# NekoImageLand/retto

Measured on AMD Instinct MI355X. Metric: images/sec end-to-end PP-OCRv4 det+rec @960x960, higher is better.
Workload: dtype f32; 1 GPU; C3: PP-OCRv4 mobile det+cls+rec full pipeline, batch=32 pages of 960x960 per GPU, 32 planted lines/page (planted DB map drives box extraction; det net fully executed, checksum 1.46374e+07); pages resident in HBM when the timed region starts; weights=seeded synthetic, PP-OCRv4 mobile shapes, networks=mobile/f32 f32 mobile/f32, parallelism=dp1 (pages sharded, no per-step collective), batches_in_flight=2

## Files before the change

include/retto_hip.h:

```cpp
#ifndef RETTO_HIP_H
#define RETTO_HIP_H

#include <stddef.h>
#include <stdint.h>

#ifdef __cplusplus
extern "C" {
#endif

#define RT_API __attribute__((visibility("default")))

typedef enum rt_status {
  RT_OK = 0,
  RT_ERR_IO = 1,
  RT_ERR_IMAGE = 2,
  RT_ERR_SHAPE = 3,
  RT_ERR_BACKEND = 4,
  RT_ERR_UTF8 = 5,
  RT_ERR_MODEL_NOT_FOUND = 7,
  RT_ERR_INVALID = 8,
  RT_ERR_CAPACITY = 9
} rt_status;

typedef struct rt_model_source {
// ... 294 lines not shown
                           int sh, int sw, const float* w, const float* bias, int act, int has_lab, float lab_a, float lab_c,
                           int pooled, int form, float* out, float* partial_out, long long partial_cap, float* mean_out,
                           int* info_out);
RT_API int rt_debug_attention(rt_session* s, const float* qkv, long long rows, const int* tokens, int n_lines, int heads,
                              float* out);
RT_API int rt_debug_lc_block(rt_session* s, const float* x, const int* heights, const int* widths, int n_img, int cin, int cout,
                             int sh, int sw, const float* dw_w, const float* dw_bias, const float* pw_w, const float* pw_bias,
                             int dw_act, int dw_has_lab, float dw_a, float dw_c, int pw_has_lab, float pw_a, float pw_c, int form,
                             float* out, int* info_out);
RT_API int rt_debug_dw_plan(int K, int sh, int sw, int Cp, int maxHo, int maxWo, int pooled, int form, int* plan_out);
RT_API int rt_debug_lc_wide(rt_session* s, const float* x, const int* heights, const int* widths, int n_img, int K, int cin, int cout,
                            int sh, int sw, const float* dw_w, const float* dw_bias, const float* pw_w, const float* pw_bias, int dw_act,
                            int dw_has_lab, float dw_a, float dw_c, int pw_has_lab, float pw_a, float pw_c, const float* fc1_w,
                            const float* fc1_b, const float* fc2_w, const float* fc2_b, int dw_form, float* out, long long out_len,
                            float* y1_out, long long y1_len, float* scale_out, long long scale_len, int* info_out);
RT_API int rt_debug_conv13(rt_session* s, const float* x, long long rows, int ldx, const int* tokens_per_line, int n_lines, int cin,
                           const float* w, int cout, const float* bias, int act, int form, float* out, int* info_out);
RT_API int rt_debug_layernorm(rt_session* s, const float* x, const float* r, long long rows, int C, const float* g,
                              const float* beta, float eps, float* out);
RT_API int rt_debug_glue16(rt_session* s, int op, const int* ip, const float* fp, const int* src_h, const int* src_w,
                           const int* dst_h, const int* dst_w, int n_img, const float* x, long long x_len, const float* x2,
                           long long x2_len, const float* tab, long long tab_len, float* out, long long out_len);
RT_API int rt_debug_fpn(rt_session* s, int op, const int* ip, const float* fp, const int* fine_h, const int* fine_w,
                        const int* coarse_h, const int* coarse_w, int n_img, const float* const* in, const long long* in_len,
                        float* const* out, const long long* out_len, int* info_out);
RT_API int rt_debug_conv16x(rt_session* s, const int* ip, const float* fp, const int* heights, const int* widths, int n_img,
                            const float* x, long long x_len, const float* wt, long long wt_len, const float* bias, const float* res,
                            long long res_len, const float* dot_w, float* out, long long out_len, int* route_out);
RT_API int rt_debug_cls_block(rt_session* s, const float* x, int n, int H, int W, int cin, int mid, int cout, int k, int sh, int act,
                              int se, const float* exp_w, const float* exp_b, const float* dw_w, const float* dw_b, const float* fc1_w,
// ... 17 lines not shown
```

retto_amd/_lib.py:

```python
from __future__ import annotations

import ctypes as C
import os

_HERE = os.path.dirname(os.path.abspath(__file__))
LIB_PATH = os.path.join(_HERE, "libretto_hip.so")

RT_OK = 0
RT_MEM_HOST, RT_MEM_DEVICE, RT_MEM_HOST_MAPS_DEVICE = 0, 1, 2
RT_MAX_INFLIGHT = 8
RT_DTYPE_F32, RT_DTYPE_F16 = 0, 1
STATUS_NAMES = {0: "OK", 1: "IOError", 2: "ImageError", 3: "ShapeError", 4: "BackendError", 5: "Utf8Error",
                7: "ModelNotFoundError", 8: "InvalidArgument", 9: "CapacityError"}


class ModelSource(C.Structure):
    _fields_ = [("path", C.c_char_p), ("data", C.c_void_p), ("len", C.c_size_t)]


class Config(C.Structure):
    _fields_ = [
        ("struct_size", C.c_uint32), ("device_id", C.c_int32),
        ("det", ModelSource), ("cls", ModelSource), ("rec", ModelSource), ("dict", ModelSource),
        ("max_side_len", C.c_int32), ("min_side_len", C.c_int32),
# ... 53 lines not shown

EXPORTS = [
    "rt_config_default", "rt_create", "rt_destroy", "rt_last_error", "rt_version",
    "rt_det", "rt_cls", "rt_rec", "rt_rec_ragged", "rt_rec_classes", "rt_model_info",
    "rt_resize_both_dims", "rt_resize_both", "rt_det_input_dims", "rt_det_preprocess", "rt_det_postprocess",
    "rt_crop_dims", "rt_crop_images", "rt_scale_and_clip", "rt_resize_norm_width", "rt_resize_norm_image",
    "rt_ctc_decode",
    "rt_run_batch", "rt_run_batch_stream", "rt_submit_batch", "rt_wait_batch", "rt_host_cpu_budget", "rt_results_free", "rt_results_pages", "rt_results_count", "rt_results_boxes",
    "rt_results_det_scores", "rt_results_cls_labels", "rt_results_cls_scores", "rt_results_rec_scores",
    "rt_results_rec_tokens", "rt_results_rec_text", "rt_results_rec_words", "rt_results_rec_word_text", "rt_debug_word_boxes", "rt_results_rec_candidates",
    "rt_debug_ctc_candidates", "rt_debug_ctc_candidates_host", "rt_results_det_checksum", "rt_results_json",
    "rt_device_malloc", "rt_device_free", "rt_memcpy_h2d", "rt_memcpy_d2h", "rt_synchronize",
    "rt_set_lanes", "rt_profile_enable", "rt_profile_get",
    "rt_onnx_to_rtwb", "rt_buffer_free", "rt_model_manifest", "rt_decode_image", "rt_run_encoded_batch",
    "rt_submit_encoded_batch", "rt_decode_batch", "rt_debug_jpeg_reconstruct",
    "rt_debug_set_variants", "rt_bench_gemm", "rt_bench_gemm_err", "rt_bench_lc", "rt_debug_conv16", "rt_debug_gemm", "rt_debug_dwconv", "rt_debug_dw_plan", "rt_debug_attention", "rt_debug_lc_block", "rt_debug_lc_wide", "rt_debug_conv13", "rt_debug_layernorm", "rt_debug_glue16", "rt_debug_conv16x", "rt_debug_fpn", "rt_debug_cls_block", "rt_debug_stem", "rt_debug_glue32", "rt_parse_dictionary", "rt_format_f32", "rt_rccl_unique_id", "rt_broadcast_blobs",
    "rt_run_regions", "rt_debug_warp_crops",
    "rt_charset_create", "rt_charset_classes", "rt_set_rec_charset", "rt_run_regions_charsets", "rt_debug_charset_compile",
    "rt_debug_ctc_charset", "rt_debug_ctc_charset_host",
    "rt_lexicon_create", "rt_lexicon_entries", "rt_lexicon_entry", "rt_lexicon_entry_text", "rt_set_rec_lexicon",
    "rt_run_regions_lexicons", "rt_results_rec_lexicon", "rt_results_rec_lexicon_id", "rt_debug_lexicon_compile",
    "rt_debug_ctc_lexicon", "rt_debug_ctc_lexicon_host",
    "rt_lexicon_set_snap", "rt_lexicon_snap", "rt_results_rec_lexicon_snapped", "rt_debug_ctc_lexicon_align",
    "rt_debug_ctc_lexicon_align_host",
    "rt_pattern_create", "rt_pattern_info", "rt_pattern_text", "rt_set_rec_pattern", "rt_run_regions_patterns", "rt_results_rec_pattern",
    "rt_debug_pattern_compile", "rt_debug_ctc_pattern", "rt_debug_ctc_pattern_host",
    "rt_keywords_create", "rt_keywords_entries", "rt_keywords_entry", "rt_keywords_entry_text", "rt_keywords_min_score",
    "rt_set_rec_keywords", "rt_run_regions_keywords", "rt_results_rec_keywords", "rt_results_rec_keywords_id", "rt_debug_ctc_keywords",
    "rt_debug_ctc_keywords_host", "rt_debug_span_quad",
    "rt_set_rec_beam", "rt_rec_beam", "rt_results_rec_beams", "rt_results_rec_beam_tokens", "rt_results_rec_beam_text",
    "rt_debug_ctc_beam", "rt_debug_ctc_beam_host",
# ... 109 lines not shown
                                        P(C.c_float), C.c_int, C.c_int, C.c_int, C.c_int, C.c_int, P(Word), P(C.c_int)]
    lib.rt_debug_gemm.argtypes = [C.c_void_p, C.c_void_p, C.c_longlong, C.c_int, C.c_int, C.c_void_p, C.c_int, C.c_void_p,
                                  C.c_int, C.c_int, C.c_float, C.c_float, C.c_void_p, C.c_int, C.c_void_p,
                                  C.c_int, C.c_void_p, C.c_int, C.c_int, C.c_int, C.c_int, C.c_int, C.c_int,
                                  C.c_void_p, C.c_void_p, C.c_void_p, C.c_void_p]
    lib.rt_debug_dwconv.argtypes = [C.c_void_p, C.c_void_p, C.c_void_p, C.c_void_p, C.c_int, C.c_int, C.c_int, C.c_int, C.c_int, C.c_int,
                                    C.c_void_p, C.c_void_p, C.c_int, C.c_int, C.c_float, C.c_float, C.c_int, C.c_int,
                                    C.c_void_p, C.c_void_p, C.c_longlong, C.c_void_p, C.c_void_p]
    lib.rt_debug_attention.argtypes = [C.c_void_p, C.c_void_p, C.c_longlong, C.c_void_p, C.c_int, C.c_int, C.c_void_p]
    lib.rt_debug_lc_block.argtypes = [C.c_void_p, C.c_void_p, C.c_void_p, C.c_void_p, C.c_int, C.c_int, C.c_int, C.c_int, C.c_int,
                                      C.c_void_p, C.c_void_p, C.c_void_p, C.c_void_p, C.c_int, C.c_int, C.c_float, C.c_float,
                                      C.c_int, C.c_float, C.c_float, C.c_int, C.c_void_p, C.c_void_p]
    lib.rt_debug_dw_plan.argtypes = [C.c_int] * 8 + [C.c_void_p]
    lib.rt_debug_lc_wide.argtypes = ([C.c_void_p] * 4 + [C.c_int] * 6 + [C.c_void_p] * 4 + [C.c_int, C.c_int, C.c_float, C.c_float, C.c_int,
                                     C.c_float, C.c_float] + [C.c_void_p] * 4 + [C.c_int] + [C.c_void_p, C.c_longlong] * 3 + [C.c_void_p])
    lib.rt_debug_conv13.argtypes = [C.c_void_p, C.c_void_p, C.c_longlong, C.c_int, C.c_void_p, C.c_int, C.c_int, C.c_void_p, C.c_int,
                                    C.c_void_p, C.c_int, C.c_int, C.c_void_p, C.c_void_p]
    lib.rt_debug_layernorm.argtypes = [C.c_void_p, C.c_void_p, C.c_void_p, C.c_longlong, C.c_int, C.c_void_p, C.c_void_p, C.c_float,
                                       C.c_void_p]
    lib.rt_debug_glue16.argtypes = [C.c_void_p, C.c_int, C.c_void_p, C.c_void_p, C.c_void_p, C.c_void_p, C.c_void_p, C.c_void_p, C.c_int,
                                    C.c_void_p, C.c_longlong, C.c_void_p, C.c_longlong, C.c_void_p, C.c_longlong, C.c_void_p,
                                    C.c_longlong]
    lib.rt_debug_fpn.argtypes = [C.c_void_p, C.c_int, C.c_void_p, C.c_void_p, C.c_void_p, C.c_void_p, C.c_void_p, C.c_void_p, C.c_int,
                                 C.c_void_p, C.c_void_p, C.c_void_p, C.c_void_p, C.c_void_p]
    lib.rt_debug_conv16x.argtypes = [C.c_void_p, C.c_void_p, C.c_void_p, C.c_void_p, C.c_void_p, C.c_int, C.c_void_p, C.c_longlong,
                                     C.c_void_p, C.c_longlong, C.c_void_p, C.c_void_p, C.c_longlong, C.c_void_p, C.c_void_p,
                                     C.c_longlong, C.c_void_p]
    lib.rt_debug_cls_block.argtypes = [C.c_void_p, C.c_void_p] + [C.c_int] * 10 + [C.c_void_p] * 10 + [C.c_int, C.c_void_p, C.c_void_p]
    lib.rt_debug_stem.argtypes = [C.c_void_p, C.c_void_p, C.c_void_p, C.c_void_p, C.c_void_p, C.c_int, C.c_int, C.c_void_p, C.c_void_p,
                                  C.c_int, C.c_float, C.c_void_p, C.c_void_p, C.c_void_p, C.c_longlong]
# ... 110 lines not shown
```

retto_amd/csrc/api_debug.cpp:

```cpp
#include <cmath>
#include <cstdio>
#include <cstdlib>
#include <cstring>

#include "api_internal.h"

using namespace rt;

namespace {
using nh::half_t;

std::vector<half_t> pack_conv16_weights(const float* wt, int cout, int cin, int kh, int kw, int cin_pad) {
  const int npad = round_up(cout, 32), nslab = (cin_pad + nh::KS - 1) / nh::KS;
  std::vector<half_t> hw((size_t)nslab * kh * kw * npad * nh::KS, (half_t)0.f);
  for (int n = 0; n < cout; n++)
    for (int k = 0; k < cin; k++)
      for (int t = 0; t < kh * kw; t++)
        hw[(((size_t)(k / nh::KS) * kh * kw + t) * npad + n) * nh::KS + k % nh::KS] = (half_t)wt[((size_t)n * cin + k) * kh * kw + t];
  return hw;
}

inline uint64_t xorshift64(uint64_t& s) { s ^= s << 13; s ^= s >> 7; s ^= s << 17; return s; }

template <typename F>
// ... 404 lines not shown
    DevBufs::download(out, dy, (size_t)out_n);
    DevBufs::download(y1_out, dy1, (size_t)y1_n);
    if (se) {
      const uint32_t cw = RT_DEBUG_CANARY;
      for (long long i = 0; i < scale_n; i++) memcpy(scale_out + i, &cw, 4);
      if (tr.scale) DevBufs::download(scale_out, tr.scale, (size_t)n_img * Cp);
    }
    const bool unfused = plan.route == nn::LC_UNFUSED;
    const int f[16] = {(int)plan.route, unfused ? (int)plan.dw.kernel : 0, unfused ? plan.dw.inst : plan.inst, plan.dw.R, plan.dw.lanes,
                       plan.dw.spb, plan.dw.chunks, (int)plan.dw.grid_x, (int)plan.dw.grid_z, plan.se_rows,
                       unfused ? (int)tr.gemm.kernel : 0, unfused && tr.gemm.se ? 1 : 0, tr.scale ? (tr.scaled_in_place ? 2 : 1) : 0, 0, 0, 0};
    memcpy(info_out, f, sizeof f);
  });
}

RT_API int rt_debug_conv13(rt_session* s, const float* x, long long rows, int ldx, const int* tokens_per_line, int n_lines, int cin,
                           const float* w, int cout, const float* bias, int act, int form, float* out, int* info_out) {
  RT_REQUIRE(s && x && tokens_per_line && w && out && info_out, s, "rt_debug_conv13: null argument");
  RT_REQUIRE(rows > 0 && rows < (1ll << 24) && n_lines > 0 && n_lines <= RT_MAX_GRID_Y && cin > 0 && cin % 4 == 0 && ldx >= cin &&
                 ldx % 4 == 0 && cout > 0 && cout <= 64 && act >= ACT_NONE && act <= ACT_SIGMOID && (form == 0 || form == 1),
             s, "rt_debug_conv13: bad shape");
  RT_REQUIRE(rows * ldx < (1ll << 30), s, "rt_debug_conv13: too large");
  for (int i = 0; i < n_lines; i++) RT_REQUIRE(tokens_per_line[i] > 0, s, "rt_debug_conv13: a line without tokens");
  const Ragged lines(tokens_per_line, n_lines);
  RT_REQUIRE(lines.total == rows, s, "rt_debug_conv13: the lines' tokens do not add up to rows");
  return guarded(s, [&] {
    RT_HIP_CHECK(hipSetDevice(s->device));
    WeightStore ws;
    const PackedDense pw = pack_conv(ws, w, bias, cout, cin, 1, 3);
    if (form == 1 && !nn::conv13_flat_supported(cout, pw.Npad)) throw RtError(RT_ERR_INVALID, "rt_debug_conv13: conv13_flat has no instance for the layer");
// ... 684 lines not shown
```

retto_amd/csrc/lc_plan.cpp:

```cpp
#include "lc_plan.h"

#include "gemm_plan.h"

namespace rt {
namespace nn {

int g_lc_wave = env_int("RT_LC_WAVE", 3);
int g_dw_sweep = env_int("RT_DW_SWEEP", 4);

namespace {

struct SweepInst { int K, sh, sw, min_ho, inst, inst_pooled; };
constexpr SweepInst SWEEPS[] = {{5, 1, 1, 5, 1, 3}, {3, 1, 1, 3, 2, 0}, {5, 2, 1, 3, 4, 5}, {3, 1, 2, 3, 6, 0}};

struct ThinInst { int sh, sw, c4, nt32, inst, th; };
constexpr ThinInst THINS[] = {{1, 1, 4, 1, 1, 8},  {1, 1, 8, 2, 2, 8},
                              {1, 1, 12, 2, 3, 4}, {1, 1, 16, 2, 4, 4},
                              {2, 2, 8, 2, 6, 4},  {2, 2, 12, 3, 7, 4}};
struct WaveInst { int sh, sw, Cp, Npad16, inst; };
constexpr WaveInst WAVES[] = {{1, 1, 16, 32, 1}, {1, 1, 32, 64, 2}, {1, 1, 48, 48, 3}, {1, 1, 64, 64, 4},
                              {2, 2, 32, 48, 6}, {2, 2, 48, 96, 7}, {2, 1, 64, 128, 8}};

int thin_inst(const LcShape& s, int* th) {
  if (s.K != 3 || s.Cp != round_up(s.C, 4)) return 0;
// ... 55 lines not shown
  };
  if (!s.se) {
    int th = 0;
    if (const int inst = g_lc_wave ? wave_inst(s, epi) : 0) {
      if (g_lc_wave >= 3 || inst >= 6) return fused(LC_LDS, inst, s.sh == 1 ? 4 : 2, 4 * LC_WAVE_TPW);
      return fused(LC_WAVE, inst, 2, 4 * LC_WAVE_TPW);
    }
    if (const int inst = thin_inst(s, &th)) return fused(LC_THIN, inst, th, LC_THIN_TPB);
  }
  if (s.se && (s.K == 3 || s.K == 5))
    p.se_rows = gemm_se_rows(s.Cp, s.rows, round_up(s.C, 4), s.N, s.Npad16, epi.act, s.min_pix);
  p.dw = dw_plan(s.K, s.sh, s.sw, s.Cp, s.maxHo, s.maxWo, p.se_rows > 0);
  return p;
}

}
}
```

retto_amd/csrc/lc_plan.h:

```cpp
#pragma once
#include "common.h"

namespace rt {
namespace nn {

extern int g_lc_wave;
extern int g_dw_sweep;

constexpr int DW_SWEEP_POOL_STRIPS = 4;
constexpr int LC_THIN_TPB = 8;
constexpr int LC_WAVE_TPW = 4;

constexpr int dw_rows_inst(int lanes, int K, int R, int sh, int sw) { return (((lanes * 8 + K) * 8 + R) * 4 + sh) * 4 + sw; }
enum class DwKernel {
  invalid,
  rows32,
  rows64,
  sweep,
};
struct DwPlan {
  DwKernel kernel = DwKernel::invalid;
  int inst = 0;
  int R = 0;
  int lanes = 0;
// ... 10 lines not shown
  int N = 0, Npad16 = 0;
  int dw_act = ACT_NONE, dw_has_lab = 0;
  bool se = false;
  int maxHo = 0, maxWo = 0, ldy = 0;
  long long rows = 0, min_pix = 0;
};
struct LcPlan {
  LcRoute route = LC_UNFUSED;
  int inst = 0, tile_h = 0;
  unsigned grid_x = 0;
  DwPlan dw;
  int se_rows = 0;
};
LcPlan lc_plan(const LcShape& s, const Epilogue& epi);

}
}
```

retto_amd/csrc/nets.cpp:

```cpp
#include "nets.h"
#include "onnx_import.h"

#include <algorithm>
#include <cstdlib>
#include <cstring>

namespace rt {

static void finish_level(Level& L) {
  long long off = 0;
  L.maxH = L.maxW = 0; L.maxPix = 0;
  for (auto& g : L.h) {
    g.off = off; g.pad_ = 0;
    off += (long long)g.H * g.W;
    L.maxH = std::max(L.maxH, g.H); L.maxW = std::max(L.maxW, g.W);
    L.maxPix = std::max(L.maxPix, (long long)g.H * g.W);
  }
  L.total = off;
}
Level make_level(const std::vector<std::pair<int, int>>& hw) {
  Level L;
  for (auto& p : hw) L.h.push_back(ImgGeom{0, p.first, p.second, 0});
  finish_level(L);
  return L;
// ... 202 lines not shown
    nn::se_scale(c.st, x, L.d, L.n(), L.maxPix, se.C, Cp, se.w1, se.b1, se.w2, se.b2, se.Cr, slope, residual, partial, scale); }
  if (apply) {
    ProfScope ps(c.prof, c.st, "scale_channels");
    nn::scale_channels(c.st, x, L.d, L.n(), L.maxPix, Cp, scale);
  }
  return scale;
}

static std::string shape_str(long long a, long long b, long long c, long long d) {
  return std::to_string(a) + "," + std::to_string(b) + "," + std::to_string(c) + "," + std::to_string(d);
}

static const float HSIG_LCNET = 0.1666667f;
static const float HSIG_MBV3 = 0.2f;

nn::LcPlan lc_block_plan(const LcBlock& b, const Level& Lout) {
  nn::LcShape s;
  s.K = b.dw.k; s.sh = b.sh; s.sw = b.sw; s.Cp = b.dw.Cp; s.C = b.dw.C; s.N = b.pw.N; s.Npad16 = b.pw.Npad;
  s.dw_act = b.dw_act; s.dw_has_lab = b.dw_lab.has; s.se = b.se;
  s.maxHo = Lout.maxH; s.maxWo = Lout.maxW; s.ldy = chan_pitch(b.cout); s.rows = Lout.total;
  s.min_pix = Lout.maxPix;
  for (const ImgGeom& g : Lout.h) s.min_pix = std::min<long long>(s.min_pix, (long long)g.H * g.W);
  return nn::lc_plan(s, make_epi(b.pw, ACT_HSWISH, &b.pw_lab));
}

float* run_lc(RunCtx& c, const LcBlock& b, const float* x, const Level& Lin, const Level& Lout, float* y2, float* y1, LcTrace* trace) {
  const nn::LcPlan plan = lc_block_plan(b, Lout);
  const int Cpo = chan_pitch(b.cout);
  Epilogue epi = make_epi(b.pw, ACT_HSWISH, &b.pw_lab);
  if (plan.route != nn::LC_UNFUSED) {
    if (!y2) y2 = c.arena->alloc<float>((size_t)Lout.total * Cpo);
    ProfScope ps(c.prof, c.st, "lc_thin", shape_str(Lout.total, b.dw.Cp, b.pw.N, b.sh * 10 + b.sw));
    (plan.route == nn::LC_THIN ? nn::lc_thin : nn::lc_wave)(c.st, plan, x, Lin.d, Lout.d, Lout.n(), b.dw.C, b.dw.w, b.dw.b, b.dw_act,
                                                            b.dw_lab.has, b.dw_lab.a, b.dw_lab.c, b.pw.w, b.pw.N, b.pw.Npad, y2, Cpo, epi);
    return y2;
  }
  if (!y1) y1 = c.arena->alloc<float>((size_t)Lout.total * b.dw.Cp);
  const nn::DwPlan& dw = plan.dw;
  const int tile_rows = plan.se_rows;
  float* pool = tile_rows ? c.arena->alloc<float>((size_t)Lout.n() * dw.chunks * b.dw.Cp) : nullptr;
  { ProfScope ps(c.prof, c.st, b.dw.k == 3 ? "dwconv3" : "dwconv5", shape_str(Lin.total, Lout.total, b.dw.Cp, b.sh * 10 + b.sw));
    nn::dwconv(c.st, dw, x, Lin.d, Lout.d, Lout.n(), b.dw.Cp, b.dw.C, b.dw.w, b.dw.b, b.dw_act, b.dw_lab.has, b.dw_lab.a, b.dw_lab.c, y1, pool); }
  if (tile_rows) {
    float* scale = c.arena->alloc<float>((size_t)Lout.n() * b.dw.Cp);
    { ProfScope ps(c.prof, c.st, "se_pool_fc");
      nn::se_fc_from_dw(c.st, pool, Lout.d, Lout.n(), dw.chunks, dw.R, dw.spb, b.sew.C, b.dw.Cp, b.sew.w1, b.sew.b1, b.sew.w2,
                        b.sew.b2, b.sew.Cr, HSIG_LCNET, 0, scale); }
    const int*& dtab = Lout.a_tabs[tile_rows];
    const int stride = tile_rows == 256 ? 3 : 2;
// ... 617 lines not shown
```

retto_amd/csrc/nets.h:

```cpp
#pragma once
#include <memory>
#include <string>
#include <map>
#include <vector>

#include "nn.h"
#include "runtime.h"

namespace rt {

struct Level {
  std::vector<ImgGeom> h;
  const ImgGeom* d = nullptr;
  long long total = 0;
  int maxH = 0, maxW = 0;
  long long maxPix = 0;
  int n() const { return (int)h.size(); }
  mutable std::map<int, const int*> a_tabs;
};

struct RunCtx {
  hipStream_t st;
  Arena* arena;
  Pinned* pinned;
  Profiler* prof;
};

Level make_level(const std::vector<std::pair<int, int>>& hw);
Level flat_level(const Level& in);
Level down_level(const Level& in, int sh, int sw);
Level pool_level(const Level& in, int kh, int kw);
void upload_levels(RunCtx& c, std::vector<Level*> levels);

// ... 35 lines not shown
Epilogue make_epi(const PackedDense& p, int act, const Lab* lab = nullptr, const float* residual = nullptr, int ld_res = 0);

struct LcBlock {
  PackedDw dw; Lab dw_lab; int dw_act = 0;
  bool se = false; SeW sew;
  PackedDense pw; Lab pw_lab;
  int sh = 1, sw = 1, cin = 0, cout = 0;
};

struct LcTrace {
  const float* scale = nullptr;
  bool scaled_in_place = false;
  nn::GemmPlan gemm;
};
nn::LcPlan lc_block_plan(const LcBlock& b, const Level& Lout);
float* run_lc(RunCtx& c, const LcBlock& b, const float* x, const Level& Lin, const Level& Lout, float* y = nullptr, float* y1 = nullptr,
              LcTrace* trace = nullptr);

struct LcSpec { const char* name; int k, cin, cout, sh, sw; bool se; };
inline constexpr LcSpec DET_SPEC[] = {
    {"s2.0", 3, 16, 32, 1, 1, false}, {"s3.0", 3, 32, 48, 2, 2, false}, {"s3.1", 3, 48, 48, 1, 1, false},
    {"s4.0", 3, 48, 96, 2, 2, false}, {"s4.1", 3, 96, 96, 1, 1, false}, {"s5.0", 3, 96, 192, 2, 2, false},
    {"s5.1", 5, 192, 192, 1, 1, false}, {"s5.2", 5, 192, 192, 1, 1, false}, {"s5.3", 5, 192, 192, 1, 1, false},
    {"s5.4", 5, 192, 192, 1, 1, false}, {"s6.0", 5, 192, 384, 2, 2, true}, {"s6.1", 5, 384, 384, 1, 1, true},
    {"s6.2", 5, 384, 384, 1, 1, false}, {"s6.3", 5, 384, 384, 1, 1, false}};
inline constexpr LcSpec REC_SPEC[] = {
    {"s2.0", 3, 16, 32, 1, 1, false}, {"s3.0", 3, 32, 64, 1, 1, false}, {"s3.1", 3, 64, 64, 1, 1, false},
    {"s4.0", 3, 64, 128, 2, 1, false}, {"s4.1", 3, 128, 128, 1, 1, false}, {"s5.0", 3, 128, 240, 1, 2, false},
    {"s5.1", 5, 240, 240, 1, 1, false}, {"s5.2", 5, 240, 240, 1, 1, false}, {"s5.3", 5, 240, 240, 1, 1, false},
    {"s5.4", 5, 240, 240, 1, 1, false}, {"s6.0", 5, 240, 480, 2, 1, true}, {"s6.1", 5, 480, 480, 1, 1, true},
// ... 110 lines not shown
```

retto_amd/csrc/nn.h:

```cpp
#pragma once
#include "common.h"
#include "gemm_plan.h"
#include "lc_plan.h"

namespace rt {
namespace nn {

constexpr int KC = 32;

void gemm(hipStream_t st, const float* A, int lda, long long M, int K, const float* Wp, int N, int Npad16, float* C,
          int ldc, int coff, const Epilogue& epi);
void gemm(hipStream_t st, const GemmPlan& p, const float* A, int lda, long long M, int K, const float* Wp, int N, int Npad16,
          float* C, int ldc, int coff, const Epilogue& epi);
void gemm_w(hipStream_t st, const float* A, int lda, long long M, int K, const float* Wp, int N, int Npad16, float* C, int ldc, int coff,
            const Epilogue& epi);
void gemm_dma(hipStream_t st, const float* A, int lda, long long M, int K, const float* Wp, int N, int Npad16, float* C,
              int ldc, int coff, const Epilogue& epi);
void gemm_split(hipStream_t st, const float* A, int lda, long long M, int K, const float* Wp, int N, int Npad16, float* C,
                int ldc, int coff, const Epilogue& epi);
void gemm_split_forget(const float* Wp);

bool conv13_flat_supported(int N, int Npad16);
void conv13_flat(hipStream_t st, const float* x, int ldx, long long rows, const unsigned char* flags, int Cin, const float* Wp, int N,
                 int Npad16, float* y, int ldy, const Epilogue& epi);
// ... 16 lines not shown

extern int g_cls_fused;
bool cls_block_supported(int k, int sh, int sw, int cin, int mid, int cout, int act, int maxH_in, int maxW, int max_pix_out);
struct ClsBlockShape { bool padrow = false; int maxu = 9, es_bytes = 0, lds = 0; };
ClsBlockShape cls_block_shape(int k, int cin, int mid, int maxH_in, int maxW, int max_pix_out);
void cls_block(hipStream_t st, int k, int sh, bool se, int act, const float* x, const ImgGeom* gin, const ImgGeom* gout, int n_img,
               int maxH_in, int maxW, int max_pix_out, int cin, int mid, int mid_cp, int cout, const float* Wexp, const float* bexp,
               const float* Wdw, const float* bdw, const float* w1, const float* b1, const float* w2, const float* b2, int cr, float slope,
               const float* Wlin, const float* blin, bool shortcut, float* y, float* dscr);
void lc_thin(hipStream_t st, const LcPlan& p, const float* x, const ImgGeom* gin, const ImgGeom* gout, int n_img, int C,
             const float* Wd, const float* bd, int dw_act, int dw_has_lab, float dw_a, float dw_c, const float* Wp, int N, int Npad16,
             float* y, int ldy, const Epilogue& epi);
void lc_wave(hipStream_t st, const LcPlan& p, const float* x, const ImgGeom* gin, const ImgGeom* gout, int n_img, int C,
             const float* Wd, const float* bd, int dw_act, int dw_has_lab, float dw_a, float dw_c, const float* Wp, int N, int Npad16,
             float* y, int ldy, const Epilogue& epi);

struct U8Page { const uint8_t* rgb; long long npix; long long out_pix; };
void stem_conv_u8(hipStream_t st, const U8Page* pages, float scale, const float* mean3, const float* std3, const ImgGeom* gin,
                  const ImgGeom* gout, int n_img, int maxHo, int maxWo, int COUT, const float* Ws, const float* bias, int act,
                  float* y);
void stem_conv(hipStream_t st, const float* x, const ImgGeom* gin, const ImgGeom* gout, int n_img, int maxHo, int maxWo,
               int COUT, const float* Ws, const float* bias, int act, float* y);

void nchw3_to_nhwc4(hipStream_t st, const float* in, int n, int H, int W, float* out);

int pool_chunks(long long max_pix);
void se_scale(hipStream_t st, const float* x, const ImgGeom* geom, int n_img, long long max_pix, int C, int Cp,
              const float* w1, const float* b1, const float* w2, const float* b2, int Cr, float slope, int residual,
              float* partial, float* scale);
void scale_channels(hipStream_t st, float* x, const ImgGeom* geom, int n_img, long long max_pix, int Cp,
// ... 58 lines not shown
```

retto_amd/csrc/nn_dev.h:

```cpp
#pragma once
#include "nn.h"

namespace rt {
namespace nn {

typedef float f32x4 __attribute__((ext_vector_type(4)));

__device__ __forceinline__ float act_apply(float v, int act) {
  if (act == ACT_HSWISH) return v * fminf(fmaxf(v + 3.0f, 0.0f), 6.0f) * 0.16666667f;
  if (act == ACT_RELU) return fmaxf(v, 0.0f);
  if (act == ACT_NONE) return v;
  const float s = __builtin_amdgcn_rcpf(1.0f + __expf(-v));
  return act == ACT_SWISH ? v * s : s;
}

template <int V> struct IntTag { static constexpr int value = V; };
template <int ACT, int LAB>
__device__ __forceinline__ float epi_val(float v, int act, int has_lab, float lab_a, float lab_c) {
  float t;
  if (ACT == ACT_HSWISH) t = v * fminf(fmaxf(v + 3.0f, 0.0f), 6.0f) * 0.16666667f;
  else if (ACT == ACT_RELU) t = fmaxf(v, 0.0f);
  else if (ACT == ACT_NONE) t = v;
  else if (ACT == ACT_SWISH) t = v * __builtin_amdgcn_rcpf(1.0f + __expf(-v));
  else t = act_apply(v, act);
  if (LAB == 1 || (LAB < 0 && has_lab)) t = fmaf(t, lab_a, lab_c);
  return t;
}
template <class F>
__device__ __forceinline__ void act_dispatch(int act, int has_lab, bool has_res, F&& f) {
  if (has_res) f(IntTag<-1>{}, IntTag<-1>{}, IntTag<1>{});
  else if (act == ACT_HSWISH && has_lab) f(IntTag<ACT_HSWISH>{}, IntTag<1>{}, IntTag<0>{});
  else if (act == ACT_HSWISH) f(IntTag<ACT_HSWISH>{}, IntTag<0>{}, IntTag<0>{});
  else if (act == ACT_NONE && !has_lab) f(IntTag<ACT_NONE>{}, IntTag<0>{}, IntTag<0>{});
  else if (act == ACT_RELU && !has_lab) f(IntTag<ACT_RELU>{}, IntTag<0>{}, IntTag<0>{});
  else if (act == ACT_SWISH && !has_lab) f(IntTag<ACT_SWISH>{}, IntTag<0>{}, IntTag<0>{});
  else f(IntTag<-1>{}, IntTag<-1>{}, IntTag<0>{});
}

}
}
```

retto_amd/csrc/nn_lcwave.hip:

```cpp
#include "common.h"
#include "nn_dev.h"

namespace rt {
namespace nn {

namespace {
constexpr int LROW = KC + 4;
constexpr int DPP_ROW_SHL1 = 0x101, DPP_ROW_SHR1 = 0x111;

template <int CTRL>
__device__ __forceinline__ f32x4 dpp_row(const f32x4& old, const f32x4& src) {
  f32x4 o;
#pragma unroll
  for (int e = 0; e < 4; e++) {
    const float fo = old[e], fs = src[e];
    o[e] = __int_as_float(__builtin_amdgcn_update_dpp(__float_as_int(fo), __float_as_int(fs), CTRL, 0xf, 0xf, false));
  }
  return o;
}
}

typedef float f32x2 __attribute__((ext_vector_type(2)));

__device__ __forceinline__ f32x4 hswish_lab4(const f32x4& v, float lab_a, float lab_c) {
  f32x4 t = v + 3.0f;
#pragma unroll
  for (int e = 0; e < 4; e++) { const float te = t[e]; t[e] = __builtin_amdgcn_fmed3f(te, 0.0f, 6.0f); }
  f32x4 o = v * t;
  o = o * 0.16666667f;
  const f32x4 a4 = {lab_a, lab_a, lab_a, lab_a}, c4 = {lab_c, lab_c, lab_c, lab_c};
  return __builtin_elementwise_fma(o, a4, c4);
}

struct LcwArgs {
  const float* x; const ImgGeom* gin; const ImgGeom* gout;
  const float* Wd; const float* bd; const float* Wp; const float* bias; float* y;
  float dw_a, dw_c, pw_a, pw_c;
  int Npad, ldy, tiles_per_wave;
};

template <int G, int NT, int MT, bool DWA>
__global__ __launch_bounds__(256) __attribute__((amdgpu_waves_per_eu(3, 3))) void k_lc_wave(LcwArgs p) {
  constexpr int CP = G * 16, NKC = (CP + KC - 1) / KC, NCOL = NT * 16;
  constexpr int IR = MT + 2;
  constexpr int NV = 2;
  __shared__ __attribute__((aligned(16))) float wt[NKC * NCOL * LROW];
// ... 322 lines not shown
```

Baseline: 1239 images/s.

## Add persistent fused depthwise3x3+pointwise kernel for 128-channel LCNet blocks

```diff
diff --git a/include/retto_hip.h b/include/retto_hip.h
--- a/include/retto_hip.h
+++ b/include/retto_hip.h
@@ -332,6 +332,9 @@
                             int dw_has_lab, float dw_a, float dw_c, int pw_has_lab, float pw_a, float pw_c, const float* fc1_w,
                             const float* fc1_b, const float* fc2_w, const float* fc2_b, int dw_form, float* out, long long out_len,
                             float* y1_out, long long y1_len, float* scale_out, long long scale_len, int* info_out);
+RT_API int rt_debug_lc_wide3(rt_session* s, const float* x, const int* heights, const int* widths, int n_img, const float* dw_w,
+                             const float* dw_bias, const float* pw_w, const float* pw_bias, float dw_a, float dw_c, float pw_a, float pw_c,
+                             float* out, long long out_len, int* info_out);
 RT_API int rt_debug_conv13(rt_session* s, const float* x, long long rows, int ldx, const int* tokens_per_line, int n_lines, int cin,
                            const float* w, int cout, const float* bias, int act, int form, float* out, int* info_out);
 RT_API int rt_debug_layernorm(rt_session* s, const float* x, const float* r, long long rows, int C, const float* g,
diff --git a/retto_amd/_lib.py b/retto_amd/_lib.py
--- a/retto_amd/_lib.py
+++ b/retto_amd/_lib.py
@@ -91,7 +91,7 @@
     "rt_set_lanes", "rt_profile_enable", "rt_profile_get",
     "rt_onnx_to_rtwb", "rt_buffer_free", "rt_model_manifest", "rt_decode_image", "rt_run_encoded_batch",
     "rt_submit_encoded_batch", "rt_decode_batch", "rt_debug_jpeg_reconstruct",
-    "rt_debug_set_variants", "rt_bench_gemm", "rt_bench_gemm_err", "rt_bench_lc", "rt_debug_conv16", "rt_debug_gemm", "rt_debug_dwconv", "rt_debug_dw_plan", "rt_debug_attention", "rt_debug_lc_block", "rt_debug_lc_wide", "rt_debug_conv13", "rt_debug_layernorm", "rt_debug_glue16", "rt_debug_conv16x", "rt_debug_fpn", "rt_debug_cls_block", "rt_debug_stem", "rt_debug_glue32", "rt_parse_dictionary", "rt_format_f32", "rt_rccl_unique_id", "rt_broadcast_blobs",
+    "rt_debug_set_variants", "rt_bench_gemm", "rt_bench_gemm_err", "rt_bench_lc", "rt_debug_conv16", "rt_debug_gemm", "rt_debug_dwconv", "rt_debug_dw_plan", "rt_debug_attention", "rt_debug_lc_block", "rt_debug_lc_wide", "rt_debug_lc_wide3", "rt_debug_conv13", "rt_debug_layernorm", "rt_debug_glue16", "rt_debug_conv16x", "rt_debug_fpn", "rt_debug_cls_block", "rt_debug_stem", "rt_debug_glue32", "rt_parse_dictionary", "rt_format_f32", "rt_rccl_unique_id", "rt_broadcast_blobs",
     "rt_run_regions", "rt_debug_warp_crops",
     "rt_charset_create", "rt_charset_classes", "rt_set_rec_charset", "rt_run_regions_charsets", "rt_debug_charset_compile",
     "rt_debug_ctc_charset", "rt_debug_ctc_charset_host",
@@ -231,6 +231,8 @@
     lib.rt_debug_dw_plan.argtypes = [C.c_int] * 8 + [C.c_void_p]
     lib.rt_debug_lc_wide.argtypes = ([C.c_void_p] * 4 + [C.c_int] * 6 + [C.c_void_p] * 4 + [C.c_int, C.c_int, C.c_float, C.c_float, C.c_int,
                                      C.c_float, C.c_float] + [C.c_void_p] * 4 + [C.c_int] + [C.c_void_p, C.c_longlong] * 3 + [C.c_void_p])
+    lib.rt_debug_lc_wide3.argtypes = ([C.c_void_p] * 4 + [C.c_int] + [C.c_void_p] * 4 + [C.c_float] * 4 +
+                                      [C.c_void_p, C.c_longlong, C.c_void_p])
     lib.rt_debug_conv13.argtypes = [C.c_void_p, C.c_void_p, C.c_longlong, C.c_int, C.c_void_p, C.c_int, C.c_int, C.c_void_p, C.c_int,
                                     C.c_void_p, C.c_int, C.c_int, C.c_void_p, C.c_void_p]
     lib.rt_debug_layernorm.argtypes = [C.c_void_p, C.c_void_p, C.c_void_p, C.c_longlong, C.c_int, C.c_void_p, C.c_void_p, C.c_float,
diff --git a/retto_amd/csrc/api_debug.cpp b/retto_amd/csrc/api_debug.cpp
--- a/retto_amd/csrc/api_debug.cpp
+++ b/retto_amd/csrc/api_debug.cpp
@@ -442,6 +442,43 @@
   });
 }
 
+RT_API int rt_debug_lc_wide3(rt_session* s, const float* x, const int* heights, const int* widths, int n_img, const float* dw_w,
+                             const float* dw_bias, const float* pw_w, const float* pw_bias, float dw_a, float dw_c, float pw_a, float pw_c,
+                             float* out, long long out_len, int* info_out) {
+  RT_REQUIRE(x && heights && widths && dw_w && dw_bias && pw_w && pw_bias && out && info_out, s, "rt_debug_lc_wide3: null argument");
+  RT_REQUIRE(n_img > 0 && n_img <= 4096, s, "rt_debug_lc_wide3: bad image count");
+  for (int i = 0; i < n_img; i++)
+    RT_REQUIRE(heights[i] > 0 && widths[i] > 0 && heights[i] <= 4096 && widths[i] <= 65536, s, "rt_debug_lc_wide3: empty or oversized image");
+  const int C = 128;
+  const Ragged gi(heights, widths, n_img);
+  RT_REQUIRE(gi.total * C < (1ll << 28), s, "rt_debug_lc_wide3: too large");
+  const long long out_n = (gi.total + 64) * C;
+  RT_REQUIRE(out_len == out_n, s, "rt_debug_lc_wide3: out has the wrong length");
+  RT_REQUIRE(s, s, "rt_debug_lc_wide3: null session");
+  return guarded(s, [&] {
+    s->begin_call();
+    WeightStore ws;
+    LcBlock b;
+    b.dw = pack_dw(ws, dw_w, dw_bias, C, 3); b.dw_lab = Lab{1, dw_a, dw_c}; b.dw_act = ACT_HSWISH;
+    b.pw = pack_conv(ws, pw_w, pw_bias, C, C, 1, 1); b.pw_lab = Lab{1, pw_a, pw_c};
+    b.sh = 1; b.sw = 1; b.cin = C; b.cout = C;
+    std::vector<std::pair<int, int>> hw;
+    for (int i = 0; i < n_img; i++) hw.push_back({heights[i], widths[i]});
+    Level Li = make_level(hw), Lo = down_level(Li, 1, 1);
+    DevBufs bufs;
+    RunCtx c = s->ctx(&s->arena);
+    upload_levels(c, {&Li, &Lo});
+    const float* dx = bufs.upload(x, (size_t)Li.total * C);
+    float* dy = bufs.canary<float>((size_t)out_n, s->st);
+    const bool fused = lc_block_wide3(b, Lo);
+    const int grid = fused ? run_lc_wide3(c, b, dx, Li, Lo, dy) : 0;
+    RT_HIP_CHECK(hipStreamSynchronize(s->st));
+    DevBufs::download(out, dy, (size_t)out_n);
+    const int f[4] = {fused ? 1 : 0, grid, Lo.wide3_tiles, stream_cus(s->st)};
+    memcpy(info_out, f, sizeof f);
+  });
+}
+
 RT_API int rt_debug_conv13(rt_session* s, const float* x, long long rows, int ldx, const int* tokens_per_line, int n_lines, int cin,
                            const float* w, int cout, const float* bias, int act, int form, float* out, int* info_out) {
   RT_REQUIRE(s && x && tokens_per_line && w && out && info_out, s, "rt_debug_conv13: null argument");
diff --git a/retto_amd/csrc/lc_plan.cpp b/retto_amd/csrc/lc_plan.cpp
--- a/retto_amd/csrc/lc_plan.cpp
+++ b/retto_amd/csrc/lc_plan.cpp
@@ -93,5 +93,29 @@
   return p;
 }
 
+int g_lc_wide3 = env_int("RT_LC_WIDE3", 1);
+
+bool lc_wide3_fused(const LcShape& s, const Epilogue& epi) {
+  if (s.K != 3 || s.sh != 1 || s.sw != 1 || s.C != 128 || s.Cp != 128 || s.N != 128 || s.Npad16 != 128 || s.ldy != 128 || s.se) return false;
+  if (s.dw_act != ACT_HSWISH || !s.dw_has_lab) return false;
+  if (epi.act != ACT_HSWISH || !epi.has_lab || !epi.bias || epi.residual || epi.a_scale || epi.am_max) return false;
+  return (long long)(s.maxHo + 2) * (s.maxWo + 2) * 128 * 4 < (1ll << 30);
+}
+
+int lc_wide3_tile_table(const ImgGeom* imgs, int n_img, int* tab) {
+  long long tiles = 0;
+  tab[0] = 0;
+  for (int i = 0; i < n_img; i++) {
+    tiles += (long long)((imgs[i].H + LC_WIDE3_TH - 1) / LC_WIDE3_TH) * ((imgs[i].W + LC_WIDE3_TW - 1) / LC_WIDE3_TW);
+    if (tiles > 0x7fffffffll) return -1;
+  }
+  tiles = 0;
+  for (int i = 0; i < n_img; i++) {
+    tiles += (long long)((imgs[i].H + LC_WIDE3_TH - 1) / LC_WIDE3_TH) * ((imgs[i].W + LC_WIDE3_TW - 1) / LC_WIDE3_TW);
+    tab[i + 1] = (int)tiles;
+  }
+  return (int)tiles;
+}
+
 }
 }
diff --git a/retto_amd/csrc/lc_plan.h b/retto_amd/csrc/lc_plan.h
--- a/retto_amd/csrc/lc_plan.h
+++ b/retto_amd/csrc/lc_plan.h
@@ -48,5 +48,10 @@
 };
 LcPlan lc_plan(const LcShape& s, const Epilogue& epi);
 
+extern int g_lc_wide3;
+constexpr int LC_WIDE3_TH = 4, LC_WIDE3_TW = 32;
+bool lc_wide3_fused(const LcShape& s, const Epilogue& epi);
+int lc_wide3_tile_table(const ImgGeom* imgs, int n_img, int* tab);
+
 }
 }
diff --git a/retto_amd/csrc/nets.cpp b/retto_amd/csrc/nets.cpp
--- a/retto_amd/csrc/nets.cpp
+++ b/retto_amd/csrc/nets.cpp
@@ -240,14 +240,32 @@
 static const float HSIG_LCNET = 0.1666667f;
 static const float HSIG_MBV3 = 0.2f;
 
-nn::LcPlan lc_block_plan(const LcBlock& b, const Level& Lout) {
+static nn::LcShape lc_block_shape(const LcBlock& b, const Level& Lout) {
   nn::LcShape s;
   s.K = b.dw.k; s.sh = b.sh; s.sw = b.sw; s.Cp = b.dw.Cp; s.C = b.dw.C; s.N = b.pw.N; s.Npad16 = b.pw.Npad;
   s.dw_act = b.dw_act; s.dw_has_lab = b.dw_lab.has; s.se = b.se;
   s.maxHo = Lout.maxH; s.maxWo = Lout.maxW; s.ldy = chan_pitch(b.cout); s.rows = Lout.total;
   s.min_pix = Lout.maxPix;
   for (const ImgGeom& g : Lout.h) s.min_pix = std::min<long long>(s.min_pix, (long long)g.H * g.W);
-  return nn::lc_plan(s, make_epi(b.pw, ACT_HSWISH, &b.pw_lab));
+  return s;
+}
+nn::LcPlan lc_block_plan(const LcBlock& b, const Level& Lout) {
+  return nn::lc_plan(lc_block_shape(b, Lout), make_epi(b.pw, ACT_HSWISH, &b.pw_lab));
+}
+bool lc_block_wide3(const LcBlock& b, const Level& Lout) {
+  return nn::lc_wide3_fused(lc_block_shape(b, Lout), make_epi(b.pw, ACT_HSWISH, &b.pw_lab));
+}
+int run_lc_wide3(RunCtx& c, const LcBlock& b, const float* x, const Level& Lin, const Level& Lout, float* y) {
+  if (!Lout.wide3_tab) {
+    int* htab = c.pinned->alloc<int>((size_t)Lout.n() + 1);
+    int* dt = c.arena->alloc<int>((size_t)Lout.n() + 1);
+    const int tiles = nn::lc_wide3_tile_table(Lout.h.data(), Lout.n(), htab);
+    if (tiles < 0) throw RtError(8, "run_lc_wide3: too many tiles");
+    RT_HIP_CHECK(hipMemcpyAsync(dt, htab, ((size_t)Lout.n() + 1) * sizeof(int), hipMemcpyHostToDevice, c.st));
+    Lout.wide3_tab = dt; Lout.wide3_tiles = tiles;
+  }
+  return nn::lc_wide3(c.st, x, Lin.d, Lout.d, Lout.wide3_tab, Lout.wide3_tiles, b.dw.w, b.dw.b, b.dw_lab.a, b.dw_lab.c, b.pw.w, y,
+                      make_epi(b.pw, ACT_HSWISH, &b.pw_lab));
 }
 
 float* run_lc(RunCtx& c, const LcBlock& b, const float* x, const Level& Lin, const Level& Lout, float* y2, float* y1, LcTrace* trace) {
@@ -259,6 +277,13 @@
     ProfScope ps(c.prof, c.st, "lc_thin", shape_str(Lout.total, b.dw.Cp, b.pw.N, b.sh * 10 + b.sw));
     (plan.route == nn::LC_THIN ? nn::lc_thin : nn::lc_wave)(c.st, plan, x, Lin.d, Lout.d, Lout.n(), b.dw.C, b.dw.w, b.dw.b, b.dw_act,
                                                             b.dw_lab.has, b.dw_lab.a, b.dw_lab.c, b.pw.w, b.pw.N, b.pw.Npad, y2, Cpo, epi);
+    return y2;
+  }
+  if (!y1 && !trace && nn::g_lc_wide3 && nn::g_gemm_variant == 0 && nn::g_gemm_split == 0 && nn::g_lc_wave == 3 && nn::g_dw_sweep == 4 &&
+      lc_block_wide3(b, Lout)) {
+    if (!y2) y2 = c.arena->alloc<float>((size_t)Lout.total * Cpo);
+    ProfScope ps(c.prof, c.st, "lc_wide3", shape_str(Lout.total, b.dw.Cp, b.pw.N, b.sh * 10 + b.sw));
+    run_lc_wide3(c, b, x, Lin, Lout, y2);
     return y2;
   }
   if (!y1) y1 = c.arena->alloc<float>((size_t)Lout.total * b.dw.Cp);
diff --git a/retto_amd/csrc/nets.h b/retto_amd/csrc/nets.h
--- a/retto_amd/csrc/nets.h
+++ b/retto_amd/csrc/nets.h
@@ -17,6 +17,8 @@
   long long maxPix = 0;
   int n() const { return (int)h.size(); }
   mutable std::map<int, const int*> a_tabs;
+  mutable const int* wide3_tab = nullptr;
+  mutable int wide3_tiles = 0;
 };
 
 struct RunCtx {
@@ -82,6 +84,8 @@
   nn::GemmPlan gemm;
 };
 nn::LcPlan lc_block_plan(const LcBlock& b, const Level& Lout);
+bool lc_block_wide3(const LcBlock& b, const Level& Lout);
+int run_lc_wide3(RunCtx& c, const LcBlock& b, const float* x, const Level& Lin, const Level& Lout, float* y);
 float* run_lc(RunCtx& c, const LcBlock& b, const float* x, const Level& Lin, const Level& Lout, float* y = nullptr, float* y1 = nullptr,
               LcTrace* trace = nullptr);
 
diff --git a/retto_amd/csrc/nn.h b/retto_amd/csrc/nn.h
--- a/retto_amd/csrc/nn.h
+++ b/retto_amd/csrc/nn.h
@@ -54,6 +54,8 @@
 void lc_wave(hipStream_t st, const LcPlan& p, const float* x, const ImgGeom* gin, const ImgGeom* gout, int n_img, int C,
              const float* Wd, const float* bd, int dw_act, int dw_has_lab, float dw_a, float dw_c, const float* Wp, int N, int Npad16,
              float* y, int ldy, const Epilogue& epi);
+int lc_wide3(hipStream_t st, const float* x, const ImgGeom* gin, const ImgGeom* gout, const int* tile0, int n_tiles, const float* Wd,
+             const float* bd, float dw_a, float dw_c, const float* Wp, float* y, const Epilogue& epi);
 
 struct U8Page { const uint8_t* rgb; long long npix; long long out_pix; };
 void stem_conv_u8(hipStream_t st, const U8Page* pages, float scale, const float* mean3, const float* std3, const ImgGeom* gin,
diff --git a/retto_amd/csrc/nn_dev.h b/retto_amd/csrc/nn_dev.h
--- a/retto_amd/csrc/nn_dev.h
+++ b/retto_amd/csrc/nn_dev.h
@@ -26,6 +26,16 @@
   if (LAB == 1 || (LAB < 0 && has_lab)) t = fmaf(t, lab_a, lab_c);
   return t;
 }
+__device__ __forceinline__ f32x4 hswish_lab4(const f32x4& v, float lab_a, float lab_c) {
+  f32x4 t = v + 3.0f;
+#pragma unroll
+  for (int e = 0; e < 4; e++) { const float te = t[e]; t[e] = __builtin_amdgcn_fmed3f(te, 0.0f, 6.0f); }
+  f32x4 o = v * t;
+  o = o * 0.16666667f;
+  const f32x4 a4 = {lab_a, lab_a, lab_a, lab_a}, c4 = {lab_c, lab_c, lab_c, lab_c};
+  return __builtin_elementwise_fma(o, a4, c4);
+}
+
 template <class F>
 __device__ __forceinline__ void act_dispatch(int act, int has_lab, bool has_res, F&& f) {
   if (has_res) f(IntTag<-1>{}, IntTag<-1>{}, IntTag<1>{});
diff --git a/retto_amd/csrc/nn_lcwave.hip b/retto_amd/csrc/nn_lcwave.hip
--- a/retto_amd/csrc/nn_lcwave.hip
+++ b/retto_amd/csrc/nn_lcwave.hip
@@ -18,18 +18,6 @@
   }
   return o;
 }
-}
-
-typedef float f32x2 __attribute__((ext_vector_type(2)));
-
-__device__ __forceinline__ f32x4 hswish_lab4(const f32x4& v, float lab_a, float lab_c) {
-  f32x4 t = v + 3.0f;
-#pragma unroll
-  for (int e = 0; e < 4; e++) { const float te = t[e]; t[e] = __builtin_amdgcn_fmed3f(te, 0.0f, 6.0f); }
-  f32x4 o = v * t;
-  o = o * 0.16666667f;
-  const f32x4 a4 = {lab_a, lab_a, lab_a, lab_a}, c4 = {lab_c, lab_c, lab_c, lab_c};
-  return __builtin_elementwise_fma(o, a4, c4);
 }
 
 struct LcwArgs {
diff --git a/retto_amd/csrc/nn_lcwide.hip b/retto_amd/csrc/nn_lcwide.hip
--- /dev/null
+++ b/retto_amd/csrc/nn_lcwide.hip
@@ -0,0 +1,229 @@
+#include <utility>
+
+#include "common.h"
+#include "lc_plan.h"
+#include "lds_asm.h"
+#include "nn_dev.h"
+
+namespace rt {
+namespace nn {
+
+namespace {
+
+struct LcWide3Args {
+  const float* x; const ImgGeom* gin; const ImgGeom* gout; const int* tile0;
+  const float* Wd; const float* bd; const float* Wp; const float* bias; float* y;
+  float dw_a, dw_c, pw_a, pw_c;
+  int n_tiles;
+};
+
+template <int... I, class F>
+__device__ __forceinline__ void static_for_impl(std::integer_sequence<int, I...>, F&& f) { (f(IntTag<I>{}), ...); }
+template <int N, class F>
+__device__ __forceinline__ void static_for(F&& f) { static_for_impl(std::make_integer_sequence<int, N>{}, f); }
+
+constexpr int X_NTHR = 512;
+constexpr int X_PW = LC_WIDE3_TW + 2, X_PIX = (LC_WIDE3_TH + 2) * X_PW;
+constexpr int X_BLK = (X_PIX + 15) / 16, X_PIECES = 2 * X_BLK;
+constexpr unsigned X_WBYTES = 128 * 128 * 4, X_SLAB = X_BLK * 2048u;
+constexpr unsigned X_TAPS = X_WBYTES + 3 * X_SLAB;
+constexpr size_t X_LDS = X_TAPS + 11 * 128 * 4;
+static_assert(LC_WIDE3_TH == 4 && LC_WIDE3_TW == 32, "8 waves = 4 rows x 2 halves of 16 columns");
+static_assert(X_PIECES > 24 && X_PIECES <= 32, "pieces wid + 8 j, j < 4; the fourth only for the first waves");
+static_assert(X_LDS <= 160 * 1024, "LDS of a CU");
+
+__global__ __launch_bounds__(X_NTHR, 1) void k_lc_wide3(const LcWide3Args g) {
+  extern __shared__ __attribute__((aligned(16))) unsigned char smemx[];
+  const int tid = threadIdx.x, lane = tid & 63;
+  const int wid = __builtin_amdgcn_readfirstlane(tid >> 6);
+  const int r = lane & 15, q = lane >> 4;
+  const int wm = wid >> 1, wh = wid & 1;
+  const unsigned lds_b = __builtin_amdgcn_readfirstlane(lds_addr(smemx));
+  float* const tp = reinterpret_cast<float*>(smemx + X_TAPS);
+  constexpr unsigned OOB = 0x80000000u;
+  const int G = gridDim.x;
+  for (int i = tid; i < 9 * 32; i += X_NTHR) reinterpret_cast<f32x4*>(tp)[i] = reinterpret_cast<const f32x4*>(g.Wd)[i];
+  if (tid < 32) reinterpret_cast<f32x4*>(tp + 9 * 128)[tid] = reinterpret_cast<const f32x4*>(g.bd)[tid];
+  else if (tid < 64) reinterpret_cast<f32x4*>(tp + 10 * 128)[tid - 32] = reinterpret_cast<const f32x4*>(g.bias)[tid - 32];
+  {
+    const int rsub = lane >> 3, c0 = lane & 7;
+    const unsigned ch = (unsigned)((c0 ^ (((rsub >> 1) | ((wid & 1) << 2)) & 7)) << 4);
+    const unsigned req_w = (unsigned)(rsub * 128) + ch;
+    const __amdgpu_buffer_rsrc_t wrs = __builtin_amdgcn_make_buffer_rsrc(const_cast<float*>(g.Wp), 0, 0x7fffffffu, 0x00020000);
+#pragma unroll
+    for (int i = 0; i < 8; i++) {
+      const unsigned p = (unsigned)(wid + 8 * i);
+      blds16(req_w, wrs, lds_b + p * 1024u, p * 1024u);
+    }
+  }
+  unsigned rq[4];
+#pragma unroll
+  for (int j = 0; j < 4; j++) {
+    const int pc = wid + 8 * j, p = 16 * (pc >> 1) + (lane & 15), chunk = 4 * (pc & 1) + (lane >> 4);
+    const int row = p / X_PW, col = p - row * X_PW;
+    rq[j] = (p < X_PIX ? (unsigned)row : 0xffu) | (unsigned)col << 8 | (unsigned)chunk << 16;
+  }
+  const int npc = wid < X_PIECES - 24 ? 4 : 3;
+  const float* xbase = nullptr;
+  unsigned xbytes = 0, goff[4];
+  auto setup_req = [&](const ImgGeom gi, int ty, int tx) __attribute__((always_inline)) {
+    const unsigned long long xa = (unsigned long long)(g.x + gi.off * 128);
+    const unsigned lo = __builtin_amdgcn_readfirstlane((unsigned)xa), hi = __builtin_amdgcn_readfirstlane((unsigned)(xa >> 32));
+    xbase = reinterpret_cast<const float*>(((unsigned long long)hi << 32) | lo);
+    xbytes = __builtin_amdgcn_readfirstlane((unsigned)gi.H * (unsigned)gi.W * 512u);
+#pragma unroll
+    for (int j = 0; j < 4; j++) {
+      const int row = rq[j] & 0xff, col = (rq[j] >> 8) & 0xff, chunk = rq[j] >> 16;
+      const int iy = ty * LC_WIDE3_TH - 1 + row, ix = tx * LC_WIDE3_TW - 1 + col;
+      const bool ok = row != 0xff && (unsigned)iy < (unsigned)gi.H && (unsigned)ix < (unsigned)gi.W;
+      goff[j] = ok ? ((unsigned)iy * (unsigned)gi.W + (unsigned)ix) * 512u + (unsigned)chunk * 16u : OOB;
+    }
+  };
+  auto issue = [&](int s, unsigned buf) __attribute__((always_inline)) {
+    const __amdgpu_buffer_rsrc_t xrs = __builtin_amdgcn_make_buffer_rsrc(const_cast<float*>(xbase), 0, xbytes, 0x00020000);
+    const unsigned dst = lds_b + X_WBYTES + buf * X_SLAB + (unsigned)wid * 1024u;
+#pragma unroll
+    for (int j = 0; j < 3; j++) blds16(goff[j], xrs, dst + j * 8192u, (unsigned)s * 128u);
+    if (npc == 4) blds16(goff[3], xrs, dst + 24576u, (unsigned)s * 128u);
+  };
+  typedef const __attribute__((address_space(4))) int* TabPtr;
+  typedef const __attribute__((address_space(4))) ImgGeom* GeomPtr;
+  const TabPtr tile0 = (TabPtr)(unsigned long long)g.tile0;
+  const GeomPtr gins = (GeomPtr)(unsigned long long)g.gin, gouts = (GeomPtr)(unsigned long long)g.gout;
+  auto geom = [](GeomPtr p) { return ImgGeom{p->off, p->H, p->W, 0}; };
+  int img = 0;
+  auto locate = [&](int t, int* ty, int* tx) __attribute__((always_inline)) {
+    while (t >= tile0[img + 1]) img++;
+    const int local = t - tile0[img], tiles_x = (gouts[img].W + LC_WIDE3_TW - 1) / LC_WIDE3_TW;
+    *ty = local / tiles_x;
+    *tx = local - *ty * tiles_x;
+  };
+  auto wait_slab = [&](bool next_slab, bool stores8) __attribute__((always_inline)) {
+    if (!next_slab) vm_wait<0>();
+    else if (stores8) { if (npc == 4) vm_wait<12>(); else vm_wait<11>(); }
+    else { if (npc == 4) vm_wait<4>(); else vm_wait<3>(); }
+  };
+  unsigned rdo[9];
+#pragma unroll
+  for (int k = 0; k < 9; k++) {
+    const int p = (wm + k / 3) * X_PW + wh * 16 + r + k % 3;
+    rdo[k] = (unsigned)((p >> 4) * 2048 + (p & 15) * 16 + q * 256);
+  }
+  const unsigned fo = lds_b + (unsigned)(r * 128) + (((unsigned)q ^ (unsigned)((r >> 1) & 7)) << 4);
+  const unsigned ta = lds_b + X_TAPS + (unsigned)q * 16u;
+
+  int t = blockIdx.x, ty, tx;
+  locate(t, &ty, &tx);
+  setup_req(geom(gins + img), ty, tx);
+  ImgGeom go = geom(gouts + img);
+  issue(0, 0u);
+  issue(1, 1u);
+  unsigned buf = 0;
+  bool stores = false;
+  for (;;) {
+    const int tn = t + G;
+    const bool more = tn < g.n_tiles;
+    const int oy = ty * LC_WIDE3_TH + wm, ox = tx * LC_WIDE3_TW + wh * 16 + r;
+    const __amdgpu_buffer_rsrc_t yrs = __builtin_amdgcn_make_buffer_rsrc(g.y + go.off * 128, 0, (unsigned)go.H * (unsigned)go.W * 512u, 0x00020000);
+    const unsigned y_off = ox < go.W ? ((unsigned)oy * (unsigned)go.W + (unsigned)ox) * 512u + (unsigned)q * 16u : OOB;
+    const bool row_ok = oy < go.H;
+    f32x4 acc[8];
+#pragma unroll
+    for (int nt = 0; nt < 8; nt++) acc[nt] = f32x4{0.f, 0.f, 0.f, 0.f};
+    static_for<4>([&](auto st) __attribute__((always_inline)) {
+      constexpr int S = decltype(st)::value;
+      wait_slab(S < 3 || more, S == 0 && stores);
+      __syncthreads();
+      if (S < 2) {
+        issue(S + 2, (buf + S + 2) % 3u);
+      } else if (more) {
+        if (S == 2) {
+          locate(tn, &ty, &tx);
+          setup_req(geom(gins + img), ty, tx);
+        }
+        issue(S - 2, (buf + S + 2) % 3u);
+      }
+      __builtin_amdgcn_sched_barrier(0);
+      const unsigned xa = lds_b + X_WBYTES + ((buf + S) % 3u) * X_SLAB;
+      unsigned pa[9];
+#pragma unroll
+      for (int k = 0; k < 9; k++) pa[k] = xa + rdo[k];
+      f32x4 v[9], w[9], d, b[8];
+      auto read_patch = [&](auto gt) __attribute__((always_inline)) {
+        static_for<9>([&](auto kt) __attribute__((always_inline)) { v[decltype(kt)::value] = lds_read16<f32x4, decltype(gt)::value * 1024>(pa[decltype(kt)::value]); });
+      };
+      auto read_taps = [&](auto gt, auto k0t, auto k1t) __attribute__((always_inline)) {
+        constexpr int GRP = decltype(gt)::value, K0 = decltype(k0t)::value, K1 = decltype(k1t)::value;
+        static_for<K1 - K0>([&](auto kt) __attribute__((always_inline)) {
+          constexpr int K = K0 + decltype(kt)::value;
+          const f32x4 t4 = lds_read16<f32x4, (K * 128 + S * 32 + GRP * 16) * 4>(ta);
+          if constexpr (K < 9) w[K] = t4; else d = t4;
+        });
+      };
+      auto read_w = [&](auto gt) __attribute__((always_inline)) {
+        static_for<8>([&](auto nt) __attribute__((always_inline)) {
+          b[decltype(nt)::value] = lds_read16<f32x4, S * 16384 + decltype(nt)::value * 2048>(decltype(gt)::value ? fo ^ 64u : fo);
+        });
+      };
+      auto mfmas = [&](f32x4 a, int nt0, int nt1) __attribute__((always_inline)) {
+#pragma unroll
+        for (int nt = nt0; nt < nt1; nt++)
+#pragma unroll
+          for (int k = 0; k < 4; k++) acc[nt] = __builtin_amdgcn_mfma_f32_16x16x4f32(b[nt][k], a[k], acc[nt], 0, 0, 0);
+        __builtin_amdgcn_sched_barrier(0);
+      };
+      auto depthwise = [&]() __attribute__((always_inline)) {
+        f32x4 dd = d;
+#pragma unroll
+        for (int k = 0; k < 9; k++) dd = __builtin_elementwise_fma(v[k], w[k], dd);
+        const f32x4 a = hswish_lab4(dd, g.dw_a, g.dw_c);
+        __builtin_amdgcn_sched_barrier(0);
+        return a;
+      };
+      read_patch(IntTag<0>{}); read_taps(IntTag<0>{}, IntTag<0>{}, IntTag<10>{});
+      read_w(IntTag<0>{});
+      lgkm_wait<8>();
+      const f32x4 a0 = depthwise();
+      read_patch(IntTag<1>{}); read_taps(IntTag<1>{}, IntTag<0>{}, IntTag<6>{});
+      lgkm_wait<15>();
+      mfmas(a0, 0, 4);
+      read_taps(IntTag<1>{}, IntTag<6>{}, IntTag<10>{});
+      __builtin_amdgcn_sched_barrier(0);
+      mfmas(a0, 4, 8);
+      read_w(IntTag<1>{});
+      lgkm_wait<8>();
+      const f32x4 a1 = depthwise();
+      lgkm_wait<0>();
+      mfmas(a1, 0, 8);
+    });
+    stores = row_ok;
+    if (row_ok) {
+#pragma unroll
+      for (int nt = 0; nt < 8; nt++) {
+        const f32x4 bias = *reinterpret_cast<const f32x4*>(tp + 10 * 128 + nt * 16 + q * 4);
+        const f32x4 o = hswish_lab4(acc[nt] + bias, g.pw_a, g.pw_c);
+        __builtin_amdgcn_raw_buffer_store_b128(__builtin_bit_cast(__attribute__((ext_vector_type(4))) unsigned, o), yrs, y_off == OOB ? OOB : y_off + nt * 64, 0, 0);
+      }
+    }
+    if (!more) break;
+    t = tn;
+    go = geom(gouts + img);
+    buf = (buf + 1) % 3u;
+  }
+}
+
+}
+
+int lc_wide3(hipStream_t st, const float* x, const ImgGeom* gin, const ImgGeom* gout, const int* tile0, int n_tiles, const float* Wd,
+             const float* bd, float dw_a, float dw_c, const float* Wp, float* y, const Epilogue& epi) {
+  if (n_tiles <= 0) return 0;
+  if (!epi.bias || epi.act != ACT_HSWISH || !epi.has_lab) throw RtError(8, "lc_wide3: the pointwise epilogue is bias + hardswish + LAB");
+  const LcWide3Args a{x, gin, gout, tile0, Wd, bd, Wp, epi.bias, y, dw_a, dw_c, epi.lab_a, epi.lab_c, n_tiles};
+  const int grid = std::min(n_tiles, stream_cus(st));
+  allow_big_lds((const void*)k_lc_wide3, 160 * 1024);
+  RT_LAUNCH(k_lc_wide3, dim3((unsigned)grid), dim3(X_NTHR), X_LDS, st, a);
+  return grid;
+}
+
+}
+}
```

Result: no change. 1249 images/s (median of 6 runs) (+0.8%).
